# foundation-model-stack/fms-fsdp

Hardware: NVIDIA H100
Metric: tokens/sec (llama2_1.4b FSDP seq4096 bs2) (higher is better)
Workload: dtype bf16; 1 GPU; model=llama2_1.4b, global_batch=2, seq_len=4096, parallelism=fsdp1, selective_ac=0, data_stream=get_dummy_loader (arange windows mod vocab, label == input), l2=per-step working set (GBs of weights+activations) >> 50 MB L2; no explicit flush

## Files before the change

### fms_fsdp_b200/csrc/attention_sm90.cu

```cuda
#include "common.cuh"
#include "tensormap.h"
#include "wgmma.cuh"

namespace b200 {

constexpr int ATT_THREADS = 256;
constexpr float LOG2E = 1.4426950408889634f;
constexpr float LN2 = 0.6931471805599453f;

template <int HD, int TB>
B200_DEVINL void mma_rs_hd(float (&d)[HD / 2], const uint32_t (&a)[4], uint64_t bdesc) {
  if constexpr (HD == 128) wgmma_bf16_rs_n128<TB>(d, a, bdesc, 1);
  else wgmma_bf16_rs_n64<TB>(d, a, bdesc, 1);
}

template <int NREG>
B200_DEVINL void acc_to_frag(const float (&v)[NREG], int kk, uint32_t (&a)[4]) {
  a[0] = pack_bf16x2(v[8 * kk + 0], v[8 * kk + 1]);
  a[1] = pack_bf16x2(v[8 * kk + 2], v[8 * kk + 3]);
  a[2] = pack_bf16x2(v[8 * kk + 4], v[8 * kk + 5]);
  a[3] = pack_bf16x2(v[8 * kk + 6], v[8 * kk + 7]);
}

B200_DEVINL float quad_max(float v) {
// ... 357 lines not shown
    }
    wgmma_commit();
    wgmma_wait<0>();
    named_bar_sync(1, ATT_THREADS);
    if (threadIdx.x == 0 && it + 2 < n_iter) load_y(it + 2);
  }

  const int Wd = (H + 2 * KVH) * HD;
#pragma unroll
  for (int hh = 0; hh < 2; ++hh) {
    const int x = x_lo + 8 * hh;
    if (x >= S) continue;
    __nv_bfloat16* drow = dqkv + ((size_t)b * S + x) * Wd;
    const int col2 = (MODE == MODE_DKDV) ? (H + kvh) * HD : head_lo * HD;
    const float* trow = rope ? rope + (size_t)x * HD : nullptr;
#pragma unroll
    for (int jj = 0; jj < HD / 8; ++jj) {
      const int c = 8 * jj + cq;
      float f0 = acc2[4 * jj + 2 * hh] * scale, f1 = acc2[4 * jj + 2 * hh + 1] * scale;
      if (trow) {
        const float2 cs = *reinterpret_cast<const float2*>(trow + c);
        const float a0 = f0, a1 = f1;
        f0 = a0 * cs.x + a1 * cs.y;
        f1 = a1 * cs.x - a0 * cs.y;
      }
      *reinterpret_cast<uint32_t*>(drow + col2 + c) = pack_bf16x2(f0, f1);
      if constexpr (MODE == MODE_DKDV)
        *reinterpret_cast<uint32_t*>(drow + (H + KVH + kvh) * HD + c) =
            pack_bf16x2(acc1[4 * jj + 2 * hh], acc1[4 * jj + 2 * hh + 1]);
    }
  }
}

template <int HD, bool DOC>
static int launch_fwd(const void* qkv, void* o, float* lse, int B, int S, int H, int KVH, float scale, const int* seg,
                      cudaStream_t st) {
  using C = FwdCfg<HD>;
  CUtensorMap tm;
  const int W = (H + 2 * KVH) * HD;
  if (make_tmap_2d_bf16(&tm, qkv, (uint64_t)W, (uint64_t)B * S, (uint64_t)W, 64, 128)) return -3;
  auto kern = attn_fwd_kernel<HD, DOC>;
  static bool configured = false;
  if (!configured) {
    cudaError_t e = cudaFuncSetAttribute(kern, cudaFuncAttributeMaxDynamicSharedMemorySize, C::SMEM);
    if (e != cudaSuccess) return (int)e;
    configured = true;
  }
  const int n_qt = (S + 127) / 128;
  kern<<<dim3(n_qt, H, B), ATT_THREADS, C::SMEM, st>>>(tm, (__nv_bfloat16*)o, lse, S, H, KVH, scale * LOG2E, n_qt,
                                                       seg);
  return (int)cudaGetLastError();
}

template <int HD, bool DOC>
static int launch_bwd(const void* dout, const void* qkv, const void* o, const float* lse, void* dqkv, float* delta,
                      int B, int S, int H, int KVH, float scale, const float* rope, const int* seg, cudaStream_t st) {
  using C = BwdCfg<HD>;
  const int W = (H + 2 * KVH) * HD;
  CUtensorMap q64, d64;
  if (make_tmap_2d_bf16(&q64, qkv, (uint64_t)W, (uint64_t)B * S, (uint64_t)W, 64, 64)) return -3;
  if (make_tmap_2d_bf16(&d64, dout, (uint64_t)H * HD, (uint64_t)B * S, (uint64_t)H * HD, 64, 64)) return -3;
  const int ld = ((S + 127) / 128) * 128;
  float* lse2 = delta + (size_t)B * H * ld;
  {
    const long long lanes = (long long)B * S * H * (HD / 8);
    const long long blocks = (lanes + 255) / 256;
    attn_delta_kernel<HD><<<(unsigned)blocks, 256, 0, st>>>((const __nv_bfloat16*)dout, (const __nv_bfloat16*)o, delta,
                                                            lse, lse2, B, S, H, ld);
  }
  auto j1 = attn_bwd_kernel<HD, MODE_DKDV, DOC>;
  auto j2 = attn_bwd_kernel<HD, MODE_DQ, DOC>;
  static bool configured = false;
  if (!configured) {
    cudaError_t e = cudaFuncSetAttribute(j1, cudaFuncAttributeMaxDynamicSharedMemorySize, C::SMEM);
    if (e != cudaSuccess) return (int)e;
    e = cudaFuncSetAttribute(j2, cudaFuncAttributeMaxDynamicSharedMemorySize, C::SMEM);
    if (e != cudaSuccess) return (int)e;
    configured = true;
  }
  const int n_t = (S + 127) / 128;
  const int* seg1 = DOC ? seg + (size_t)B * S : nullptr;
  j1<<<dim3(n_t, KVH, B), ATT_THREADS, C::SMEM, st>>>(q64, d64, lse2, delta, (__nv_bfloat16*)dqkv, S, H, KVH, scale, n_t,
                                                      ld, rope, seg1);
  j2<<<dim3(n_t, H, B), ATT_THREADS, C::SMEM, st>>>(q64, d64, lse2, delta, (__nv_bfloat16*)dqkv, S, H, KVH, scale, n_t,
                                                    ld, rope, seg);
  return (int)cudaGetLastError();
}

}

extern "C" int b200_attn_fwd(const void* qkv, void* o, float* lse, int B, int S, int H, int KVH, int HD, float scale,
                             cudaStream_t st, const int* seg) {
  if (H % KVH) return -1;
  if (seg) {
    if (HD == 128) return b200::launch_fwd<128, true>(qkv, o, lse, B, S, H, KVH, scale, seg, st);
    if (HD == 64) return b200::launch_fwd<64, true>(qkv, o, lse, B, S, H, KVH, scale, seg, st);
    return -2;
  }
  if (HD == 128) return b200::launch_fwd<128, false>(qkv, o, lse, B, S, H, KVH, scale, nullptr, st);
  if (HD == 64) return b200::launch_fwd<64, false>(qkv, o, lse, B, S, H, KVH, scale, nullptr, st);
  return -2;
}
extern "C" int b200_attn_bwd(const void* dout, const void* qkv, const void* o, const float* lse, void* dqkv,
                             float* delta, int B, int S, int H, int KVH, int HD, float scale, const float* rope,
                             cudaStream_t st, const int* seg) {
  if (H % KVH) return -1;
  if (seg) {
    if (HD == 128) return b200::launch_bwd<128, true>(dout, qkv, o, lse, dqkv, delta, B, S, H, KVH, scale, rope, seg, st);
    if (HD == 64) return b200::launch_bwd<64, true>(dout, qkv, o, lse, dqkv, delta, B, S, H, KVH, scale, rope, seg, st);
    return -2;
  }
  if (HD == 128) return b200::launch_bwd<128, false>(dout, qkv, o, lse, dqkv, delta, B, S, H, KVH, scale, rope, nullptr, st);
  if (HD == 64) return b200::launch_bwd<64, false>(dout, qkv, o, lse, dqkv, delta, B, S, H, KVH, scale, rope, nullptr, st);
  return -2;
}
```

### fms_fsdp_b200/csrc/bindings.cpp

```cpp
#include <ATen/cuda/CUDAContext.h>
#include <c10/cuda/CUDAGuard.h>
#include <torch/extension.h>

#include <cmath>
#include <cstdint>

#define DECL extern "C"
DECL int b200_gemm_bf16(const void*, const void*, void*, const void*, int, int, int, int, int, int, int, int, int, int,
                        int, cudaStream_t);
DECL int b200_gemm2_bf16(const void*, const void*, void*, const void*, int, int, int, int, int, int, int, int, int, int,
                         int, cudaStream_t);
DECL int b200_gemm2_ag_bf16(const void*, const void*, void*, const void*, int, int, int, int, int, int, int, int, int, int,
                            const void* const*, void*, unsigned long long, unsigned long long, unsigned long long, int, int,
                            uint32_t*, uint32_t, int, cudaStream_t);
DECL int b200_bgemm_bf16(const void*, const void*, void*, int, int, int, int, int, int, int, int, long long, long long,
                         long long, long long, long long, long long, int, int, int, int, cudaStream_t);
DECL int b200_ssd_prep(const void*, const float*, const float*, float*, float*, float*, int, int, int, cudaStream_t);
DECL int b200_ssd_mask(const void*, const float*, const float*, void*, int, int, int, cudaStream_t);
DECL int b200_ssd_xs(const void*, const float*, const float*, const float*, void*, long long, int, int, cudaStream_t);
DECL int b200_ssd_state_pass(const float*, const float*, void*, int, int, int, int, int, cudaStream_t);
DECL int b200_ssd_combine(const void*, const void*, const void*, const float*, const float*, void*, long long, int, int,
                          cudaStream_t);
DECL int b200_ssd_dyoff(const void*, const void*, const void*, const float*, void*, float*, float*, long long, int,
                        cudaStream_t);
// ... 8 lines not shown
DECL int b200_selscan_fwd(const void*, const void*, const float*, const void*, const void*, const float*, const void*,
                          const float*, float*, void*, int, int, int, int, int, cudaStream_t);
DECL int b200_selscan_bwd(const void*, const void*, const void*, const float*, const void*, const void*, const float*,
                          const void*, const float*, float*, void*, void*, void*, float*, float*, float*, float*, float*, int,
                          int, int, int, int, cudaStream_t);
DECL void b200_comm_set_reduce_ctas(int);
DECL int b200_p2p_gather_range(const void* const*, void*, long long, long long, long long, cudaStream_t);
DECL int b200_rmsnorm_fwd(const void*, const void*, void*, float*, int, int, float, cudaStream_t);
DECL int b200_rmsnorm_bwd_grid(int);
DECL int b200_rmsnorm_bwd(const void*, const void*, const void*, const float*, const void*, void*, float*, float*, int, int,
                          cudaStream_t);
DECL int b200_add_rmsnorm_fwd(const void*, const float*, const void*, void*, float*, float*, int, int, float, cudaStream_t);
DECL int b200_rmsnorm_bwd_f32(const void*, const float*, const void*, const float*, float*, float*, float*, int, int, cudaStream_t);
DECL int b200_rmsnorm_gated_fwd(const void*, const void*, const void*, void*, float*, int, int, float, cudaStream_t);
DECL int b200_rmsnorm_gated_bwd(const void*, const void*, const void*, const void*, const float*, void*, void*, float*, float*, int, int, cudaStream_t);
DECL int b200_rope(void*, const float*, int, int, int, int, int, int, int, int, int, cudaStream_t);
DECL int b200_qk_norm_rope(void*, void*, float*, const void*, const void*, const float*, int, int, int, int, int, int, float,
                           cudaStream_t);
DECL int b200_qk_norm_bwd_grid(int, int, int);
DECL int b200_qk_norm_bwd(void*, const void*, const float*, const void*, const void*, float*, float*, int, int, int, int,
                          int, cudaStream_t);
DECL int b200_swiglu_fwd(const void*, void*, long long, int, int, cudaStream_t);
DECL int b200_swiglu_bwd(const void*, const void*, void*, long long, int, int, cudaStream_t);
DECL int b200_embedding_fwd(const void*, int, const void*, void*, long long, int, cudaStream_t);
DECL int b200_embedding_bwd(const void*, int, const void*, void*, int, long long, int, cudaStream_t);
DECL int b200_count_valid(const long long*, int, long long, float*, cudaStream_t);
DECL int b200_ce_grad_inplace(void*, const long long*, const float*, float*, int, int, int, long long, cudaStream_t);
DECL int b200_adamw(float*, const void*, int, float*, float*, void*, long long, float, float, float, float, float,
                    float, float, const float*, cudaStream_t);
DECL int b200_sumsq(const void*, int, long long, float*, cudaStream_t);
DECL int b200_attn_fwd(const void*, void*, float*, int, int, int, int, int, float, cudaStream_t, const int*);
DECL int b200_attn_bwd(const void*, const void*, const void*, const float*, void*, float*, int, int, int, int, int,
                       float, const float*, cudaStream_t, const int*);
DECL void b200_gemm2_set_rope(const float*, int, int, int);
DECL void b200_gemm2_set_swiglu(void*, int, int, int);
DECL void b200_gemm2_set_tile(int);
DECL int b200_gemm2_fp8(const void*, const void*, void*, const float*, const float*, int, int, int, int, int, int, cudaStream_t);
DECL int b200_quant_rowwise_e4m3(const void*, void*, float*, int, int, int, int, cudaStream_t);
DECL void b200_gemm2_set_push(void* const*, long long, long long, int, int, int);
DECL int b200_p2p_push_range(const void*, void* const*, long long, long long, long long, int, cudaStream_t);
DECL int b200_p2p_allgather(const void* const*, void*, long long, int, int, cudaStream_t);
DECL int b200_reduce_scatter(const void* const*, float*, long long, long long, int, int, int, float, float*, int,
                             cudaStream_t);
DECL int b200_allreduce_inplace(void* const*, long long, int, int, int, float, float*, cudaStream_t);
DECL int b200_signal_barrier(uint32_t* const*, int, int, uint32_t, int, int, cudaStream_t);
DECL int b200_scalar_allreduce_bytes();
DECL int b200_scalar_allreduce(uint8_t* const*, int, int, uint32_t, float*, int, cudaStream_t);
DECL int b200_gemm_grouped_bf16(const void*, const void*, void*, const int*, const int*, int, int, int, int, int, int, int,
                                int, int, int, int, cudaStream_t);
DECL int b200_moe_route(const float*, int, int, int, int, float*, int*, float*, cudaStream_t);
DECL int b200_moe_plan_ws_chunks(int);
DECL int b200_moe_plan(const int*, const float*, int, int, int, int, int*, float*, int*, int*, int*, int*, int*, float*,
                       cudaStream_t);
DECL int b200_moe_permute(const void*, const int*, const int*, const int*, const int*, int, int, int, void*, cudaStream_t);
DECL int b200_moe_permute_bwd(const void*, const int*, int, int, int, void*, cudaStream_t);
DECL int b200_moe_combine(const void*, const int*, const float*, const void*, int, int, int, void*, cudaStream_t);
DECL int b200_moe_combine_bwd(const void*, const void*, const float*, const int*, const int*, const int*, const int*, int,
                              int, int, void*, float*, cudaStream_t);
DECL int b200_moe_route_bwd(const float*, const int*, const float*, const float*, const int*, int, int, int, int, float,
                            void*, cudaStream_t);
DECL int b200_causal_conv1d_fwd(const void*, const void*, const void*, void*, int, int, int, int, int, cudaStream_t);
DECL int b200_causal_conv1d_bwd(const void*, const void*, const void*, const void*, void*, float*, float*, int, int,
                                int, int, int, cudaStream_t);

namespace {

// ... 278 lines not shown
  need(master, "master", at::kFloat);
  need(m, "m", at::kFloat);
  need(v, "v", at::kFloat);
  TORCH_CHECK(grad.scalar_type() == at::kBFloat16 || grad.scalar_type() == at::kFloat);
  TORCH_CHECK(grad.numel() == master.numel());
  void* lp = nullptr;
  if (lowp.has_value()) {
    need(*lowp, "lowp", at::kBFloat16);
    lp = lowp->data_ptr();
  }
  const float* gs = grad_scale.has_value() ? grad_scale->data_ptr<float>() : nullptr;
  const double bc1 = 1.0 - std::pow(b1, (double)step), bc2 = 1.0 - std::pow(b2, (double)step);
  check(b200_adamw(master.data_ptr<float>(), grad.data_ptr(), grad.scalar_type() == at::kBFloat16,
                   m.data_ptr<float>(), v.data_ptr<float>(), lp, master.numel(), (float)lr, (float)b1, (float)b2,
                   (float)eps, (float)wd, (float)bc1, (float)std::sqrt(bc2), gs, cur_stream()), "adamw");
}
void sumsq(const at::Tensor& x, at::Tensor& out) {
  c10::cuda::CUDAGuard guard(x.device());
  TORCH_CHECK(x.is_contiguous() && (x.scalar_type() == at::kBFloat16 || x.scalar_type() == at::kFloat));
  need(out, "out", at::kFloat);
  check(b200_sumsq(x.data_ptr(), x.scalar_type() == at::kBFloat16, x.numel(), out.data_ptr<float>(), cur_stream()),
        "sumsq");
}

const int* seg_ptr(const c10::optional<at::Tensor>& seg, const at::Tensor& qkv, int64_t B, int64_t S) {
  if (!seg.has_value() || !seg->defined()) return nullptr;
  TORCH_CHECK(seg->scalar_type() == at::kInt, "seg has dtype ", seg->scalar_type(), ", expected int32");
  TORCH_CHECK(seg->is_contiguous(), "seg must be contiguous");
  TORCH_CHECK(seg->device() == qkv.device(), "seg must be on the device of qkv");
  TORCH_CHECK(seg->numel() == 2 * B * S, "seg must be a [2, B*S] table");
  return seg->data_ptr<int>();
}

std::vector<at::Tensor> attn_fwd(const at::Tensor& qkv, int64_t B, int64_t S, int64_t H, int64_t KVH, int64_t hd,
                                 double scale, const c10::optional<at::Tensor>& seg) {
  c10::cuda::CUDAGuard guard(qkv.device());
  need(qkv, "qkv", at::kBFloat16);
  TORCH_CHECK(qkv.is_contiguous());
  const int* seg_p = seg_ptr(seg, qkv, B, S);
  auto o = at::empty({B * S, H * hd}, qkv.options());
  auto lse = at::empty({B, H, S}, qkv.options().dtype(at::kFloat));
  check(b200_attn_fwd(qkv.data_ptr(), o.data_ptr(), lse.data_ptr<float>(), B, S, H, KVH, hd, (float)scale,
                      cur_stream(), seg_p), "attn_fwd");
  return {o, lse};
}
at::Tensor attn_bwd(const at::Tensor& dout, const at::Tensor& qkv, const at::Tensor& o, const at::Tensor& lse,
                    int64_t B, int64_t S, int64_t H, int64_t KVH, int64_t hd, double scale,
                    const c10::optional<at::Tensor>& rope, const c10::optional<at::Tensor>& seg) {
  c10::cuda::CUDAGuard guard(qkv.device());
  need(qkv, "qkv", at::kBFloat16);
  need(dout, "do", at::kBFloat16);
  need(o, "o", at::kBFloat16);
  need(lse, "lse", at::kFloat);
  TORCH_CHECK(qkv.is_contiguous() && dout.is_contiguous() && o.is_contiguous() && lse.is_contiguous());
  const int* seg_p = seg_ptr(seg, qkv, B, S);
  auto dqkv = at::empty_like(qkv);
  auto delta = at::empty({2, B, H, ((S + 127) / 128) * 128}, qkv.options().dtype(at::kFloat));
  const float* rope_p = nullptr;
  if (rope.has_value() && rope->defined()) {
    need(*rope, "rope", at::kFloat);
    TORCH_CHECK(rope->is_contiguous() && rope->numel() >= S * hd, "attn_bwd: rope table must be [S, hd/2, 2] fp32");
    rope_p = rope->data_ptr<float>();
  }
  check(b200_attn_bwd(dout.data_ptr(), qkv.data_ptr(), o.data_ptr(), lse.data_ptr<float>(), dqkv.data_ptr(),
                      delta.data_ptr<float>(), B, S, H, KVH, hd, (float)scale, rope_p, cur_stream(), seg_p),
        "attn_bwd", 3);
  return dqkv;
}

void p2p_allgather(const at::Tensor& peer_ptrs, at::Tensor& full, int64_t shard_bytes, int64_t world, int64_t rank) {
  c10::cuda::CUDAGuard guard(full.device());
  check(b200_p2p_allgather((const void* const*)peer_ptrs.data_ptr(), full.data_ptr(), shard_bytes, world, rank,
                           cur_stream()), "p2p_allgather");
}
void reduce_scatter(const at::Tensor& peer_ptrs, at::Tensor& out32, int64_t elem_offset, int64_t world, int64_t rank,
                    bool src_bf16, double scale, const c10::optional<at::Tensor>& sumsq_out, int64_t max_ctas,
                    bool accumulate) {
  c10::cuda::CUDAGuard guard(out32.device());
  need(out32, "out", at::kFloat);
  b200_comm_set_reduce_ctas(max_ctas > 0 ? (int)max_ctas : g_reduce_ctas_default);
  check(b200_reduce_scatter((const void* const*)peer_ptrs.data_ptr(), out32.data_ptr<float>(), out32.numel(),
                            elem_offset, world, rank, src_bf16, (float)scale,
                            sumsq_out.has_value() ? sumsq_out->data_ptr<float>() : nullptr, accumulate ? 1 : 0,
                            cur_stream()),
        "reduce_scatter");
}
void allreduce_inplace(const at::Tensor& peer_ptrs, int64_t numel, int64_t world, int64_t rank, bool is_bf16,
                       double scale, const c10::optional<at::Tensor>& sumsq_out, const at::Tensor& anchor) {
  c10::cuda::CUDAGuard guard(anchor.device());
  check(b200_allreduce_inplace((void* const*)peer_ptrs.data_ptr(), numel, world, rank, is_bf16, (float)scale,
                               sumsq_out.has_value() ? sumsq_out->data_ptr<float>() : nullptr, cur_stream()),
        "allreduce_inplace");
}
void signal_barrier(const at::Tensor& pad_ptrs, int64_t world, int64_t rank, int64_t epoch, const at::Tensor& anchor,
                    int64_t slot_base, int64_t mode) {
  c10::cuda::CUDAGuard guard(anchor.device());
  check(b200_signal_barrier((uint32_t* const*)pad_ptrs.data_ptr(), world, rank, (uint32_t)epoch, (int)slot_base, (int)mode,
                            cur_stream()), "signal_barrier");
}
void scalar_allreduce(const at::Tensor& buf_ptrs, int64_t world, int64_t rank, int64_t epoch, at::Tensor& inout) {
// ... 490 lines not shown
PYBIND11_MODULE(TORCH_EXTENSION_NAME, m) {
  m.doc() = "fms_fsdp_b200 sm_90a kernels";
  m.def("gemm", &gemm);
  m.def("gemm_grouped", &gemm_grouped);
  m.def("moe_route", &moe_route);
  m.def("moe_plan", &moe_plan);
  m.def("moe_permute", &moe_permute);
  m.def("moe_permute_bwd", &moe_permute_bwd);
  m.def("moe_combine", &moe_combine);
  m.def("moe_combine_bwd", &moe_combine_bwd);
  m.def("moe_route_bwd", &moe_route_bwd);
  m.def("rmsnorm_fwd", &rmsnorm_fwd);
  m.def("rmsnorm_bwd", &rmsnorm_bwd, py::arg("dy"), py::arg("x"), py::arg("w"), py::arg("rstd"), py::arg("dres") = py::none());
  m.def("add_rmsnorm_fwd", &add_rmsnorm_fwd);
  m.def("rmsnorm_bwd_f32", &rmsnorm_bwd_f32);
  m.def("rmsnorm_gated_fwd", &rmsnorm_gated_fwd);
  m.def("rmsnorm_gated_bwd", &rmsnorm_gated_bwd);
  m.def("rope", &rope);
  m.def("qk_norm_rope", &qk_norm_rope);
  m.def("qk_norm_bwd", &qk_norm_bwd);
  m.def("swiglu_fwd", &swiglu_fwd);
  m.def("swiglu_bwd", &swiglu_bwd);
  m.def("embedding_fwd", &embedding_fwd);
  m.def("embedding_bwd", &embedding_bwd);
  m.def("count_valid", &count_valid);
  m.def("ce_grad_inplace", &ce_grad_inplace);
  m.def("adamw", &adamw);
  m.def("sumsq", &sumsq);
  m.def("attn_fwd", &attn_fwd, py::arg("qkv"), py::arg("B"), py::arg("S"), py::arg("H"), py::arg("KVH"), py::arg("hd"),
        py::arg("scale"), py::arg("seg") = py::none());
  m.def("attn_bwd", &attn_bwd, py::arg("dout"), py::arg("qkv"), py::arg("o"), py::arg("lse"), py::arg("B"), py::arg("S"),
        py::arg("H"), py::arg("KVH"), py::arg("hd"), py::arg("scale"), py::arg("rope") = py::none(),
        py::arg("seg") = py::none());
  m.def("p2p_allgather", &p2p_allgather);
  m.def("reduce_scatter", &reduce_scatter, py::arg("peer_ptrs"), py::arg("out32"), py::arg("elem_offset"), py::arg("world"),
        py::arg("rank"), py::arg("src_bf16"), py::arg("scale"), py::arg("sumsq_out"), py::arg("max_ctas") = 0,
        py::arg("accumulate") = false);
  m.def("allreduce_inplace", &allreduce_inplace);
  m.def("signal_barrier", &signal_barrier, py::arg("pad_ptrs"), py::arg("world"), py::arg("rank"), py::arg("epoch"),
        py::arg("anchor"), py::arg("slot_base") = 0, py::arg("mode") = 0);
  m.def("scalar_allreduce", &scalar_allreduce);
  m.def("scalar_allreduce_bytes", []() { return (int64_t)b200_scalar_allreduce_bytes(); });
  m.def("causal_conv1d_fwd", &causal_conv1d_fwd);
  m.def("causal_conv1d_bwd", &causal_conv1d_bwd);
  m.def("set_reduce_ctas", [](int64_t n) { g_reduce_ctas_default = n < 1 ? 1 : (int)n; b200_comm_set_reduce_ctas((int)n); });
  m.def("set_gemm_rope", [](const at::Tensor& table, int64_t S, int64_t hd, int64_t cols) {
    need(table, "rope table", at::kFloat);
    TORCH_CHECK(table.is_contiguous() && table.numel() >= S * hd, "rope table must be [S, hd/2, 2] fp32");
    b200_gemm2_set_rope(table.data_ptr<float>(), (int)S, (int)hd, (int)cols);
  });
  m.def("push_range", [](const at::Tensor& src, const at::Tensor& bases, int64_t n, int64_t off, int64_t rank) {
    c10::cuda::CUDAGuard guard(src.device());
    need(src, "src", at::kBFloat16);
    TORCH_CHECK(src.is_contiguous() && bases.scalar_type() == at::kLong && bases.is_cuda());
    check(b200_p2p_push_range(src.data_ptr(), (void* const*)bases.data_ptr(), n, off, src.numel(), (int)rank, cur_stream()),
          "p2p_push_range");
  });
  m.def("set_gemm_swiglu", [](const at::Tensor& aux, int64_t F, bool gate_first) {
    need(aux, "aux", at::kBFloat16);
    TORCH_CHECK(aux.dim() == 2 && aux.stride(1) == 1 && (aux.size(1) == F || aux.size(1) == 2 * F));
    b200_gemm2_set_swiglu(aux.data_ptr(), (int)aux.stride(0), (int)F, gate_first ? 1 : 0);
  });
  m.def("set_gemm_push", [](const at::Tensor& bases, int64_t n, int64_t off, int64_t rank, bool bulk, int64_t rot_world) {
    TORCH_CHECK(bases.is_cuda() && bases.scalar_type() == at::kLong && bases.is_contiguous(), "push table: int64 CUDA tensor");
    b200_gemm2_set_push((void* const*)bases.data_ptr(), n, off, (int)rank, bulk ? 1 : 0, (int)rot_world);
  }, py::arg("bases"), py::arg("n"), py::arg("off"), py::arg("rank"), py::arg("bulk") = true, py::arg("rot_world") = 1);
// ... 16 lines not shown
```

Baseline: 49640 tokens/s.

## Add warp-specialized TMA producer/consumer pipelined attention forward and backward kernels

Adds new forward and backward attention kernels that dedicate one warpgroup to TMA loads (with setmaxnreg register reallocation) and two consumer warpgroups that run wgmma. K/V tiles are multi-buffered with full/empty mbarriers, and the forward overlaps the next QK^T with the current PV product. The default entry points now dispatch to the pipelined path, and the old kernels stay reachable through new lockstep bindings. This is meant to hide load latency and keep the tensor cores busy, at the cost of higher shared-memory and register pressure and one CTA per SM.

Result: faster. 52770 tokens/s, median of 6 (+6.3%).

```diff
diff --git a/fms_fsdp_b200/csrc/attention_sm90.cu b/fms_fsdp_b200/csrc/attention_sm90.cu
--- a/fms_fsdp_b200/csrc/attention_sm90.cu
+++ b/fms_fsdp_b200/csrc/attention_sm90.cu
@@ -413,30 +413,464 @@
   }
 }
 
+constexpr int PIPE_THREADS = 384;
+constexpr int PRODUCER_REGS = 24, CONSUMER_REGS = 240;
+
+template <int N>
+B200_DEVINL void attn_regs_dec() { asm volatile("setmaxnreg.dec.sync.aligned.u32 %0;" ::"n"(N)); }
+template <int N>
+B200_DEVINL void attn_regs_inc() { asm volatile("setmaxnreg.inc.sync.aligned.u32 %0;" ::"n"(N)); }
+
+B200_DEVINL void bulk_load_1d(void* dst, const void* src, uint32_t bytes, uint64_t* bar) {
+  asm volatile("cp.async.bulk.shared::cluster.global.mbarrier::complete_tx::bytes [%0], [%1], %2, [%3];"
+               ::"r"(smem_u32(dst)), "l"(reinterpret_cast<uint64_t>(src)), "r"(bytes), "r"(smem_u32(bar))
+               : "memory");
+}
+
+template <int HD>
+struct FwdPipeCfg {
+  static constexpr int NCH = HD / 64;
+  static constexpr int TILE_BYTES = 128 * HD * 2;
+  static constexpr int STAGES = 2;
+  static constexpr int SMEM = TILE_BYTES * (1 + 2 * STAGES) + 1024 + 256;
+};
+
 template <int HD, bool DOC>
+__global__ void __launch_bounds__(PIPE_THREADS, 1)
+attn_fwd_pipe_kernel(const __grid_constant__ CUtensorMap tm, __nv_bfloat16* __restrict__ o, float* __restrict__ lse,
+                     int S, int H, int KVH, float scale_log2, int n_qt, const int* __restrict__ seg0) {
+  using C = FwdPipeCfg<HD>;
+  constexpr int ST = C::STAGES;
+  extern __shared__ uint8_t smem_raw[];
+  uint8_t* smem = reinterpret_cast<uint8_t*>((reinterpret_cast<uintptr_t>(smem_raw) + 1023) & ~uintptr_t(1023));
+  uint8_t* sQ = smem;
+  uint8_t* sK = sQ + C::TILE_BYTES;
+  uint8_t* sV = sK + ST * C::TILE_BYTES;
+  uint64_t* bars = reinterpret_cast<uint64_t*>(sV + ST * C::TILE_BYTES);
+  uint64_t* q_full = bars;
+  uint64_t* k_full = bars + 1;
+  uint64_t* v_full = k_full + ST;
+  uint64_t* k_empty = v_full + ST;
+  uint64_t* v_empty = k_empty + ST;
+
+  const int wg = threadIdx.x >> 7, w4 = (threadIdx.x >> 5) & 3, lane = threadIdx.x & 31;
+  const int h = blockIdx.x, b = blockIdx.y;
+  const int qt = n_qt - 1 - blockIdx.z;
+  const int kvh = h / (H / KVH);
+  const int row0 = b * S + qt * 128;
+  const int n_kv = min(qt + 1, (S + 127) / 128);
+  const int* srow = DOC ? seg0 + static_cast<size_t>(b) * S : nullptr;
+  const int j_lo = DOC ? srow[qt * 128] / 128 : 0;
+
+  if (threadIdx.x == 0) {
+    mbar_init(q_full, 1);
+    for (int s = 0; s < ST; ++s) {
+      mbar_init(&k_full[s], 1);
+      mbar_init(&v_full[s], 1);
+      mbar_init(&k_empty[s], 8);
+      mbar_init(&v_empty[s], 8);
+    }
+    fence_barrier_init();
+  }
+  __syncthreads();
+
+  if (wg == 0) {
+    attn_regs_dec<PRODUCER_REGS>();
+    if (threadIdx.x == 0) {
+      tma_prefetch_desc(&tm);
+      mbar_arrive_expect_tx(q_full, C::TILE_BYTES);
+      for (int c = 0; c < C::NCH; ++c) tma_load_2d(sQ + c * 16384, &tm, q_full, h * HD + 64 * c, row0);
+      for (int j = j_lo; j < n_kv; ++j) {
+        const int st = (j - j_lo) % ST;
+        const uint32_t ph = ((j - j_lo) / ST) & 1;
+        const int krow = b * S + j * 128;
+        mbar_wait(&k_empty[st], ph ^ 1);
+        mbar_arrive_expect_tx(&k_full[st], C::TILE_BYTES);
+        for (int c = 0; c < C::NCH; ++c)
+          tma_load_2d(sK + st * C::TILE_BYTES + c * 16384, &tm, &k_full[st], (H + kvh) * HD + 64 * c, krow);
+        mbar_wait(&v_empty[st], ph ^ 1);
+        mbar_arrive_expect_tx(&v_full[st], C::TILE_BYTES);
+        for (int c = 0; c < C::NCH; ++c)
+          tma_load_2d(sV + st * C::TILE_BYTES + c * 16384, &tm, &v_full[st], (H + KVH + kvh) * HD + 64 * c, krow);
+      }
+    }
+    asm volatile("exit;");
+  }
+  attn_regs_inc<CONSUMER_REGS>();
+  const int cw = wg - 1;
+
+  const int r_lo = qt * 128 + cw * 64 + w4 * 16 + (lane >> 2);
+  const int cq = 2 * (lane & 3);
+  int doc_lo[2] = {0, 0}, tile_doc_hi = 0;
+  if constexpr (DOC) {
+    doc_lo[0] = srow[min(r_lo, S - 1)];
+    doc_lo[1] = srow[min(r_lo + 8, S - 1)];
+    tile_doc_hi = srow[min(qt * 128 + 127, S - 1)];
+  }
+  const uint64_t qd = make_smem_desc(smem_u32(sQ) + cw * 8192, 0, 1024);
+  float oacc[HD / 2];
+#pragma unroll
+  for (int i = 0; i < HD / 2; ++i) oacc[i] = 0.f;
+  float m_run[2] = {-INFINITY, -INFINITY}, l_run[2] = {0.f, 0.f};
+
+  auto issue_s = [&](int j, float (&s)[64]) {
+    const int n = j - j_lo;
+    mbar_wait(&k_full[n % ST], (n / ST) & 1);
+    const uint64_t kd = make_smem_desc(smem_u32(sK + (n % ST) * C::TILE_BYTES), 0, 1024);
+    wgmma_fence();
+#pragma unroll
+    for (int kk = 0; kk < HD / 16; ++kk) {
+      const uint32_t off = ((kk >> 2) * 16384 + (kk & 3) * 32) >> 4;
+      wgmma_bf16_ss_n128<0, 0>(s, qd + off, kd + off, kk != 0);
+    }
+    wgmma_commit();
+  };
+  auto issue_pv = [&](int j, const uint32_t (&pa)[8][4]) {
+    const int n = j - j_lo;
+    mbar_wait(&v_full[n % ST], (n / ST) & 1);
+    const uint64_t vd = make_smem_desc(smem_u32(sV + (n % ST) * C::TILE_BYTES), 16384, 1024);
+    wgmma_fence();
+#pragma unroll
+    for (int kk = 0; kk < 8; ++kk) mma_rs_hd<HD, 1>(oacc, pa[kk], vd + ((kk * 2048) >> 4));
+    wgmma_commit();
+  };
+  auto release = [&](uint64_t* empty, int j) {
+    if (lane == 0) mbar_arrive(&empty[(j - j_lo) % ST]);
+  };
+  auto softmax = [&](int j, float (&s)[64], float (&corr)[2]) {
+    const int kv0 = j * 128;
+    if (j == qt || kv0 + 128 > S || (DOC && kv0 < tile_doc_hi)) {
+#pragma unroll
+      for (int i = 0; i < 64; ++i) {
+        const int kv = kv0 + 8 * (i >> 2) + cq + (i & 1);
+        const int q = r_lo + 8 * ((i >> 1) & 1);
+        if (kv > q || kv >= S || (DOC && kv < doc_lo[(i >> 1) & 1])) s[i] = -INFINITY;
+      }
+    }
+#pragma unroll
+    for (int hh = 0; hh < 2; ++hh) {
+      float mx = -INFINITY;
+#pragma unroll
+      for (int jj = 0; jj < 16; ++jj) mx = fmaxf(mx, fmaxf(s[4 * jj + 2 * hh], s[4 * jj + 2 * hh + 1]));
+      const float m_new = fmaxf(m_run[hh], quad_max(mx) * scale_log2);
+      const float m_sub = (DOC && m_new == -INFINITY) ? 0.f : m_new;
+      corr[hh] = exp2f(m_run[hh] - m_sub);
+      m_run[hh] = m_new;
+      float ls = 0.f;
+#pragma unroll
+      for (int jj = 0; jj < 16; ++jj) {
+#pragma unroll
+        for (int e = 0; e < 2; ++e) {
+          const int i = 4 * jj + 2 * hh + e;
+          s[i] = exp2f(fmaf(s[i], scale_log2, -m_sub));
+          ls += s[i];
+        }
+      }
+      l_run[hh] = l_run[hh] * corr[hh] + ls;
+    }
+  };
+
+  mbar_wait(q_full, 0);
+  float s[64], corr[2];
+  uint32_t pa[8][4];
+  issue_s(j_lo, s);
+  wgmma_wait<0>();
+  release(k_empty, j_lo);
+  softmax(j_lo, s, corr);
+#pragma unroll
+  for (int i = 0; i < HD / 2; ++i) oacc[i] *= corr[(i >> 1) & 1];
+#pragma unroll
+  for (int kk = 0; kk < 8; ++kk) acc_to_frag(s, kk, pa[kk]);
+  for (int j = j_lo + 1; j < n_kv; ++j) {
+    issue_s(j, s);
+    issue_pv(j - 1, pa);
+    wgmma_wait<1>();
+    release(k_empty, j);
+    softmax(j, s, corr);
+    wgmma_wait<0>();
+    release(v_empty, j - 1);
+#pragma unroll
+    for (int i = 0; i < HD / 2; ++i) oacc[i] *= corr[(i >> 1) & 1];
+#pragma unroll
+    for (int kk = 0; kk < 8; ++kk) acc_to_frag(s, kk, pa[kk]);
+  }
+  issue_pv(n_kv - 1, pa);
+  wgmma_wait<0>();
+
+#pragma unroll
+  for (int hh = 0; hh < 2; ++hh) {
+    const int q = r_lo + 8 * hh;
+    const float l = quad_sum(l_run[hh]);
+    if (q < S) {
+      const float inv_l = 1.f / l;
+      __nv_bfloat16* orow = o + (static_cast<size_t>(b) * S + q) * (H * HD) + h * HD;
+#pragma unroll
+      for (int jj = 0; jj < HD / 8; ++jj)
+        *reinterpret_cast<uint32_t*>(orow + 8 * jj + cq) =
+            pack_bf16x2(oacc[4 * jj + 2 * hh] * inv_l, oacc[4 * jj + 2 * hh + 1] * inv_l);
+      if ((lane & 3) == 0) lse[(static_cast<size_t>(b) * H + h) * S + q] = (m_run[hh] + log2f(l)) * LN2;
+    }
+  }
+}
+
+template <int HD>
+struct BwdPipeCfg {
+  static constexpr int NCH = HD / 64;
+  static constexpr int X_BYTES = 128 * HD * 2;
+  static constexpr int Y_BYTES = 64 * HD * 2;
+  static constexpr int STAGES = 3;
+  static constexpr int STAT_BYTES = 2 * 64 * 4;
+  static constexpr int SMEM = 2 * X_BYTES + STAGES * (2 * Y_BYTES + STAT_BYTES) + 1024 + 256;
+};
+
+template <int HD, int MODE, bool DOC>
+__global__ void __launch_bounds__(PIPE_THREADS, 1)
+attn_bwd_pipe_kernel(const __grid_constant__ CUtensorMap tm_qkv, const __grid_constant__ CUtensorMap tm_do,
+                     const float* __restrict__ lse2g, const float* __restrict__ delta, __nv_bfloat16* __restrict__ dqkv,
+                     int S, int H, int KVH, float scale, int n_t128, int ld, const float* __restrict__ rope,
+                     const int* __restrict__ seg_plane) {
+  using C = BwdPipeCfg<HD>;
+  constexpr int ST = C::STAGES;
+  extern __shared__ uint8_t smem_raw[];
+  uint8_t* smem = reinterpret_cast<uint8_t*>((reinterpret_cast<uintptr_t>(smem_raw) + 1023) & ~uintptr_t(1023));
+  uint8_t* sX1 = smem;
+  uint8_t* sX2 = sX1 + C::X_BYTES;
+  uint8_t* sY = sX2 + C::X_BYTES;
+  float* sStat = reinterpret_cast<float*>(sY + ST * 2 * C::Y_BYTES);
+  uint64_t* bars = reinterpret_cast<uint64_t*>(sStat + ST * 128);
+  uint64_t* x_full = bars;
+  uint64_t* y_full = bars + 1;
+  uint64_t* y_empty = y_full + ST;
+
+  const int wg = threadIdx.x >> 7, w4 = (threadIdx.x >> 5) & 3, lane = threadIdx.x & 31;
+  const int G = H / KVH;
+  const int b = blockIdx.y;
+  const float scale_log2 = scale * LOG2E;
+  const int n_t64 = (S + 63) / 64;
+  int t128, head_lo, head_n, kvh;
+  if constexpr (MODE == MODE_DKDV) {
+    t128 = blockIdx.z; kvh = blockIdx.x; head_lo = kvh * G; head_n = G;
+  } else {
+    t128 = n_t128 - 1 - blockIdx.z; head_lo = blockIdx.x; head_n = 1; kvh = blockIdx.x / G;
+  }
+  const int* srow = DOC ? seg_plane + static_cast<size_t>(b) * S : nullptr;
+  const int tile_doc_first = DOC ? srow[t128 * 128] : 0;
+  const int tile_doc_last = DOC ? srow[min(t128 * 128 + 127, S - 1)] : 0;
+  const int s_lo = (MODE == MODE_DKDV) ? 2 * t128 : (DOC ? tile_doc_first / 64 : 0);
+  const int s_hi = (MODE == MODE_DKDV) ? (DOC ? tile_doc_last / 64 + 1 : n_t64) : min(2 * t128 + 2, n_t64);
+  const int per_head = s_hi - s_lo;
+  const int n_iter = per_head * head_n;
+  const int xrow0 = b * S + t128 * 128;
+
+  if (threadIdx.x == 0) {
+    mbar_init(x_full, 1);
+    for (int s = 0; s < ST; ++s) {
+      mbar_init(&y_full[s], 1);
+      mbar_init(&y_empty[s], 8);
+    }
+    fence_barrier_init();
+  }
+  __syncthreads();
+
+  if (wg == 0) {
+    attn_regs_dec<PRODUCER_REGS>();
+    if (threadIdx.x == 0) {
+      tma_prefetch_desc(&tm_qkv); tma_prefetch_desc(&tm_do);
+      mbar_arrive_expect_tx(x_full, 2 * C::X_BYTES);
+      for (int c = 0; c < C::NCH; ++c) {
+        for (int half = 0; half < 2; ++half) {
+          uint8_t* d1 = sX1 + c * 16384 + half * 8192;
+          uint8_t* d2 = sX2 + c * 16384 + half * 8192;
+          const int r = xrow0 + 64 * half;
+          if constexpr (MODE == MODE_DKDV) {
+            tma_load_2d(d1, &tm_qkv, x_full, (H + kvh) * HD + 64 * c, r);
+            tma_load_2d(d2, &tm_qkv, x_full, (H + KVH + kvh) * HD + 64 * c, r);
+          } else {
+            tma_load_2d(d1, &tm_qkv, x_full, head_lo * HD + 64 * c, r);
+            tma_load_2d(d2, &tm_do, x_full, head_lo * HD + 64 * c, r);
+          }
+        }
+      }
+      for (int it = 0; it < n_iter; ++it) {
+        const int st = it % ST;
+        const int hh = head_lo + it / per_head;
+        const int y0 = (s_lo + it % per_head) * 64;
+        uint8_t* y1 = sY + st * 2 * C::Y_BYTES;
+        uint8_t* y2 = y1 + C::Y_BYTES;
+        mbar_wait(&y_empty[st], ((it / ST) & 1) ^ 1);
+        mbar_arrive_expect_tx(&y_full[st], 2 * C::Y_BYTES + (MODE == MODE_DKDV ? C::STAT_BYTES : 0));
+        for (int c = 0; c < C::NCH; ++c) {
+          if constexpr (MODE == MODE_DKDV) {
+            tma_load_2d(y1 + c * 8192, &tm_qkv, &y_full[st], hh * HD + 64 * c, b * S + y0);
+            tma_load_2d(y2 + c * 8192, &tm_do, &y_full[st], hh * HD + 64 * c, b * S + y0);
+          } else {
+            tma_load_2d(y1 + c * 8192, &tm_qkv, &y_full[st], (H + kvh) * HD + 64 * c, b * S + y0);
+            tma_load_2d(y2 + c * 8192, &tm_qkv, &y_full[st], (H + KVH + kvh) * HD + 64 * c, b * S + y0);
+          }
+        }
+        if constexpr (MODE == MODE_DKDV) {
+          const size_t base = ((size_t)b * H + hh) * ld + y0;
+          bulk_load_1d(sStat + st * 128, lse2g + base, 256, &y_full[st]);
+          bulk_load_1d(sStat + st * 128 + 64, delta + base, 256, &y_full[st]);
+        }
+      }
+    }
+    asm volatile("exit;");
+  }
+  attn_regs_inc<CONSUMER_REGS>();
+  const int cw = wg - 1;
+
+  const int x_lo = t128 * 128 + cw * 64 + w4 * 16 + (lane >> 2);
+  const int cq = 2 * (lane & 3);
+  const uint64_t x1d = make_smem_desc(smem_u32(sX1) + cw * 8192, 0, 1024);
+  const uint64_t x2d = make_smem_desc(smem_u32(sX2) + cw * 8192, 0, 1024);
+  float acc1[MODE == MODE_DKDV ? HD / 2 : 1];
+  float acc2[HD / 2];
+#pragma unroll
+  for (int i = 0; i < HD / 2; ++i) acc2[i] = 0.f;
+#pragma unroll
+  for (int i = 0; i < (MODE == MODE_DKDV ? HD / 2 : 1); ++i) acc1[i] = 0.f;
+  float row_nl[2] = {0.f, 0.f}, row_nd[2] = {0.f, 0.f};
+  int row_doc[2] = {0, 0};
+  if constexpr (DOC) {
+    row_doc[0] = srow[min(x_lo, S - 1)];
+    row_doc[1] = srow[min(x_lo + 8, S - 1)];
+  }
+  if constexpr (MODE == MODE_DQ) {
+#pragma unroll
+    for (int hh = 0; hh < 2; ++hh) {
+      const size_t sidx = ((size_t)b * H + head_lo) * ld + min(x_lo + 8 * hh, S - 1);
+      row_nl[hh] = lse2g[sidx];
+      row_nd[hh] = delta[sidx];
+    }
+  }
+
+  constexpr bool CARRY = !(MODE == MODE_DKDV && HD == 128);
+  mbar_wait(x_full, 0);
+  uint32_t pa[4][4], da[4][4];
+  for (int it = 0; it < n_iter; ++it) {
+    const int st = it % ST;
+    const int y0 = (s_lo + it % per_head) * 64;
+    const uint32_t y1a = smem_u32(sY + st * 2 * C::Y_BYTES), y2a = y1a + C::Y_BYTES;
+    mbar_wait(&y_full[st], (it / ST) & 1);
+    const uint64_t y1d = make_smem_desc(y1a, 0, 1024), y2d = make_smem_desc(y2a, 0, 1024);
+    float s[32], dp[32];
+    wgmma_fence();
+#pragma unroll
+    for (int kk = 0; kk < HD / 16; ++kk) {
+      const uint32_t ox = ((kk >> 2) * 16384 + (kk & 3) * 32) >> 4, oy = ((kk >> 2) * 8192 + (kk & 3) * 32) >> 4;
+      wgmma_bf16_ss_n64<0, 0>(s, x1d + ox, y1d + oy, kk != 0);
+    }
+    wgmma_commit();
+#pragma unroll
+    for (int kk = 0; kk < HD / 16; ++kk) {
+      const uint32_t ox = ((kk >> 2) * 16384 + (kk & 3) * 32) >> 4, oy = ((kk >> 2) * 8192 + (kk & 3) * 32) >> 4;
+      wgmma_bf16_ss_n64<0, 0>(dp, x2d + ox, y2d + oy, kk != 0);
+    }
+    wgmma_commit();
+    wgmma_wait<1>();
+    if (CARRY && it > 0 && lane == 0) mbar_arrive(&y_empty[(it - 1) % ST]);
+    const bool diag = (MODE == MODE_DKDV) ? (y0 < t128 * 128 + 128) : (y0 + 64 > t128 * 128);
+    const bool doc_edge = DOC && ((MODE == MODE_DKDV) ? (y0 + 63 > tile_doc_first) : (y0 < tile_doc_last));
+    const bool need_mask = diag || (y0 + 64 > S) || (t128 * 128 + 128 > S) || doc_edge;
+    const float* stl = sStat + st * 128;
+    uint32_t mbits = 0;
+#pragma unroll
+    for (int i = 0; i < 32; ++i) {
+      const int x = x_lo + 8 * ((i >> 1) & 1);
+      const int y = y0 + 8 * (i >> 2) + cq + (i & 1);
+      const float nl = (MODE == MODE_DKDV) ? stl[8 * (i >> 2) + cq + (i & 1)] : row_nl[(i >> 1) & 1];
+      bool masked = false;
+      if (need_mask) masked = (MODE == MODE_DKDV) ? (x > y || y >= S || x >= S) : (y > x || y >= S || x >= S);
+      if constexpr (DOC) {
+        const int bound = row_doc[(i >> 1) & 1];
+        if (need_mask) masked = masked || ((MODE == MODE_DKDV) ? (y > bound) : (y < bound));
+      }
+      mbits |= (masked ? 1u : 0u) << i;
+      s[i] = masked ? 0.f : exp2f(fmaf(s[i], scale_log2, nl));
+    }
+    const uint64_t y1t = make_smem_desc(y1a, 8192, 1024), y2t = make_smem_desc(y2a, 8192, 1024);
+    if constexpr (MODE == MODE_DKDV) {
+#pragma unroll
+      for (int kk = 0; kk < 4; ++kk) acc_to_frag(s, kk, pa[kk]);
+      wgmma_fence();
+#pragma unroll
+      for (int kk = 0; kk < 4; ++kk) mma_rs_hd<HD, 1>(acc1, pa[kk], y2t + ((kk * 2048) >> 4));
+      wgmma_commit();
+      wgmma_wait<1>();
+    } else {
+      wgmma_wait<0>();
+    }
+#pragma unroll
+    for (int i = 0; i < 32; ++i) {
+      const float nd = (MODE == MODE_DKDV) ? stl[64 + 8 * (i >> 2) + cq + (i & 1)] : row_nd[(i >> 1) & 1];
+      dp[i] = ((mbits >> i) & 1u) ? 0.f : s[i] * (dp[i] + nd);
+    }
+#pragma unroll
+    for (int kk = 0; kk < 4; ++kk) acc_to_frag(dp, kk, da[kk]);
+    wgmma_fence();
+#pragma unroll
+    for (int kk = 0; kk < 4; ++kk) mma_rs_hd<HD, 1>(acc2, da[kk], y1t + ((kk * 2048) >> 4));
+    wgmma_commit();
+    if constexpr (!CARRY) {
+      wgmma_wait<0>();
+      if (lane == 0) mbar_arrive(&y_empty[st]);
+    }
+  }
+  wgmma_wait<0>();
+
+  const int Wd = (H + 2 * KVH) * HD;
+#pragma unroll
+  for (int hh = 0; hh < 2; ++hh) {
+    const int x = x_lo + 8 * hh;
+    if (x >= S) continue;
+    __nv_bfloat16* drow = dqkv + ((size_t)b * S + x) * Wd;
+    const int col2 = (MODE == MODE_DKDV) ? (H + kvh) * HD : head_lo * HD;
+    const float* trow = rope ? rope + (size_t)x * HD : nullptr;
+#pragma unroll
+    for (int jj = 0; jj < HD / 8; ++jj) {
+      const int c = 8 * jj + cq;
+      float f0 = acc2[4 * jj + 2 * hh] * scale, f1 = acc2[4 * jj + 2 * hh + 1] * scale;
+      if (trow) {
+        const float2 cs = *reinterpret_cast<const float2*>(trow + c);
+        const float a0 = f0, a1 = f1;
+        f0 = a0 * cs.x + a1 * cs.y;
+        f1 = a1 * cs.x - a0 * cs.y;
+      }
+      *reinterpret_cast<uint32_t*>(drow + col2 + c) = pack_bf16x2(f0, f1);
+      if constexpr (MODE == MODE_DKDV)
+        *reinterpret_cast<uint32_t*>(drow + (H + KVH + kvh) * HD + c) =
+            pack_bf16x2(acc1[4 * jj + 2 * hh], acc1[4 * jj + 2 * hh + 1]);
+    }
+  }
+}
+
+template <int HD, bool DOC, bool PIPE>
 static int launch_fwd(const void* qkv, void* o, float* lse, int B, int S, int H, int KVH, float scale, const int* seg,
                       cudaStream_t st) {
-  using C = FwdCfg<HD>;
+  constexpr int SMEM = PIPE ? FwdPipeCfg<HD>::SMEM : FwdCfg<HD>::SMEM;
   CUtensorMap tm;
   const int W = (H + 2 * KVH) * HD;
   if (make_tmap_2d_bf16(&tm, qkv, (uint64_t)W, (uint64_t)B * S, (uint64_t)W, 64, 128)) return -3;
-  auto kern = attn_fwd_kernel<HD, DOC>;
+  auto kern = PIPE ? attn_fwd_pipe_kernel<HD, DOC> : attn_fwd_kernel<HD, DOC>;
   static bool configured = false;
   if (!configured) {
-    cudaError_t e = cudaFuncSetAttribute(kern, cudaFuncAttributeMaxDynamicSharedMemorySize, C::SMEM);
+    cudaError_t e = cudaFuncSetAttribute(kern, cudaFuncAttributeMaxDynamicSharedMemorySize, SMEM);
     if (e != cudaSuccess) return (int)e;
     configured = true;
   }
   const int n_qt = (S + 127) / 128;
-  kern<<<dim3(n_qt, H, B), ATT_THREADS, C::SMEM, st>>>(tm, (__nv_bfloat16*)o, lse, S, H, KVH, scale * LOG2E, n_qt,
-                                                       seg);
+  if constexpr (PIPE)
+    kern<<<dim3(H, B, n_qt), PIPE_THREADS, SMEM, st>>>(tm, (__nv_bfloat16*)o, lse, S, H, KVH, scale * LOG2E, n_qt, seg);
+  else
+    kern<<<dim3(n_qt, H, B), ATT_THREADS, SMEM, st>>>(tm, (__nv_bfloat16*)o, lse, S, H, KVH, scale * LOG2E, n_qt, seg);
   return (int)cudaGetLastError();
 }
 
-template <int HD, bool DOC>
+template <int HD, bool DOC, bool PIPE>
 static int launch_bwd(const void* dout, const void* qkv, const void* o, const float* lse, void* dqkv, float* delta,
                       int B, int S, int H, int KVH, float scale, const float* rope, const int* seg, cudaStream_t st) {
-  using C = BwdCfg<HD>;
+  constexpr int SMEM = PIPE ? BwdPipeCfg<HD>::SMEM : BwdCfg<HD>::SMEM;
   const int W = (H + 2 * KVH) * HD;
   CUtensorMap q64, d64;
   if (make_tmap_2d_bf16(&q64, qkv, (uint64_t)W, (uint64_t)B * S, (uint64_t)W, 64, 64)) return -3;
@@ -449,49 +883,70 @@
     attn_delta_kernel<HD><<<(unsigned)blocks, 256, 0, st>>>((const __nv_bfloat16*)dout, (const __nv_bfloat16*)o, delta,
                                                             lse, lse2, B, S, H, ld);
   }
-  auto j1 = attn_bwd_kernel<HD, MODE_DKDV, DOC>;
-  auto j2 = attn_bwd_kernel<HD, MODE_DQ, DOC>;
+  auto j1 = PIPE ? attn_bwd_pipe_kernel<HD, MODE_DKDV, DOC> : attn_bwd_kernel<HD, MODE_DKDV, DOC>;
+  auto j2 = PIPE ? attn_bwd_pipe_kernel<HD, MODE_DQ, DOC> : attn_bwd_kernel<HD, MODE_DQ, DOC>;
   static bool configured = false;
   if (!configured) {
-    cudaError_t e = cudaFuncSetAttribute(j1, cudaFuncAttributeMaxDynamicSharedMemorySize, C::SMEM);
+    cudaError_t e = cudaFuncSetAttribute(j1, cudaFuncAttributeMaxDynamicSharedMemorySize, SMEM);
     if (e != cudaSuccess) return (int)e;
-    e = cudaFuncSetAttribute(j2, cudaFuncAttributeMaxDynamicSharedMemorySize, C::SMEM);
+    e = cudaFuncSetAttribute(j2, cudaFuncAttributeMaxDynamicSharedMemorySize, SMEM);
     if (e != cudaSuccess) return (int)e;
     configured = true;
   }
   const int n_t = (S + 127) / 128;
   const int* seg1 = DOC ? seg + (size_t)B * S : nullptr;
-  j1<<<dim3(n_t, KVH, B), ATT_THREADS, C::SMEM, st>>>(q64, d64, lse2, delta, (__nv_bfloat16*)dqkv, S, H, KVH, scale, n_t,
-                                                      ld, rope, seg1);
-  j2<<<dim3(n_t, H, B), ATT_THREADS, C::SMEM, st>>>(q64, d64, lse2, delta, (__nv_bfloat16*)dqkv, S, H, KVH, scale, n_t,
-                                                    ld, rope, seg);
+  const dim3 g1 = PIPE ? dim3(KVH, B, n_t) : dim3(n_t, KVH, B), g2 = PIPE ? dim3(H, B, n_t) : dim3(n_t, H, B);
+  const int threads = PIPE ? PIPE_THREADS : ATT_THREADS;
+  j1<<<g1, threads, SMEM, st>>>(q64, d64, lse2, delta, (__nv_bfloat16*)dqkv, S, H, KVH, scale, n_t, ld, rope, seg1);
+  j2<<<g2, threads, SMEM, st>>>(q64, d64, lse2, delta, (__nv_bfloat16*)dqkv, S, H, KVH, scale, n_t, ld, rope, seg);
   return (int)cudaGetLastError();
+}
+
+template <bool PIPE>
+static int attn_fwd(const void* qkv, void* o, float* lse, int B, int S, int H, int KVH, int HD, float scale,
+                    cudaStream_t st, const int* seg) {
+  if (H % KVH) return -1;
+  if (seg) {
+    if (HD == 128) return launch_fwd<128, true, PIPE>(qkv, o, lse, B, S, H, KVH, scale, seg, st);
+    if (HD == 64) return launch_fwd<64, true, PIPE>(qkv, o, lse, B, S, H, KVH, scale, seg, st);
+    return -2;
+  }
+  if (HD == 128) return launch_fwd<128, false, PIPE>(qkv, o, lse, B, S, H, KVH, scale, nullptr, st);
+  if (HD == 64) return launch_fwd<64, false, PIPE>(qkv, o, lse, B, S, H, KVH, scale, nullptr, st);
+  return -2;
+}
+
+template <bool PIPE>
+static int attn_bwd(const void* dout, const void* qkv, const void* o, const float* lse, void* dqkv, float* delta, int B,
+                    int S, int H, int KVH, int HD, float scale, const float* rope, cudaStream_t st, const int* seg) {
+  if (H % KVH) return -1;
+  if (seg) {
+    if (HD == 128) return launch_bwd<128, true, PIPE>(dout, qkv, o, lse, dqkv, delta, B, S, H, KVH, scale, rope, seg, st);
+    if (HD == 64) return launch_bwd<64, true, PIPE>(dout, qkv, o, lse, dqkv, delta, B, S, H, KVH, scale, rope, seg, st);
+    return -2;
+  }
+  if (HD == 128) return launch_bwd<128, false, PIPE>(dout, qkv, o, lse, dqkv, delta, B, S, H, KVH, scale, rope, nullptr, st);
+  if (HD == 64) return launch_bwd<64, false, PIPE>(dout, qkv, o, lse, dqkv, delta, B, S, H, KVH, scale, rope, nullptr, st);
+  return -2;
 }
 
 }
 
 extern "C" int b200_attn_fwd(const void* qkv, void* o, float* lse, int B, int S, int H, int KVH, int HD, float scale,
                              cudaStream_t st, const int* seg) {
-  if (H % KVH) return -1;
-  if (seg) {
-    if (HD == 128) return b200::launch_fwd<128, true>(qkv, o, lse, B, S, H, KVH, scale, seg, st);
-    if (HD == 64) return b200::launch_fwd<64, true>(qkv, o, lse, B, S, H, KVH, scale, seg, st);
-    return -2;
-  }
-  if (HD == 128) return b200::launch_fwd<128, false>(qkv, o, lse, B, S, H, KVH, scale, nullptr, st);
-  if (HD == 64) return b200::launch_fwd<64, false>(qkv, o, lse, B, S, H, KVH, scale, nullptr, st);
-  return -2;
+  return b200::attn_fwd<true>(qkv, o, lse, B, S, H, KVH, HD, scale, st, seg);
 }
 extern "C" int b200_attn_bwd(const void* dout, const void* qkv, const void* o, const float* lse, void* dqkv,
                              float* delta, int B, int S, int H, int KVH, int HD, float scale, const float* rope,
                              cudaStream_t st, const int* seg) {
-  if (H % KVH) return -1;
-  if (seg) {
-    if (HD == 128) return b200::launch_bwd<128, true>(dout, qkv, o, lse, dqkv, delta, B, S, H, KVH, scale, rope, seg, st);
-    if (HD == 64) return b200::launch_bwd<64, true>(dout, qkv, o, lse, dqkv, delta, B, S, H, KVH, scale, rope, seg, st);
-    return -2;
-  }
-  if (HD == 128) return b200::launch_bwd<128, false>(dout, qkv, o, lse, dqkv, delta, B, S, H, KVH, scale, rope, nullptr, st);
-  if (HD == 64) return b200::launch_bwd<64, false>(dout, qkv, o, lse, dqkv, delta, B, S, H, KVH, scale, rope, nullptr, st);
-  return -2;
-}
+  return b200::attn_bwd<true>(dout, qkv, o, lse, dqkv, delta, B, S, H, KVH, HD, scale, rope, st, seg);
+}
+extern "C" int b200_attn_fwd_lockstep(const void* qkv, void* o, float* lse, int B, int S, int H, int KVH, int HD,
+                                      float scale, cudaStream_t st, const int* seg) {
+  return b200::attn_fwd<false>(qkv, o, lse, B, S, H, KVH, HD, scale, st, seg);
+}
+extern "C" int b200_attn_bwd_lockstep(const void* dout, const void* qkv, const void* o, const float* lse, void* dqkv,
+                                      float* delta, int B, int S, int H, int KVH, int HD, float scale, const float* rope,
+                                      cudaStream_t st, const int* seg) {
+  return b200::attn_bwd<false>(dout, qkv, o, lse, dqkv, delta, B, S, H, KVH, HD, scale, rope, st, seg);
+}
diff --git a/fms_fsdp_b200/csrc/bindings.cpp b/fms_fsdp_b200/csrc/bindings.cpp
--- a/fms_fsdp_b200/csrc/bindings.cpp
+++ b/fms_fsdp_b200/csrc/bindings.cpp
@@ -64,6 +64,9 @@
 DECL int b200_attn_fwd(const void*, void*, float*, int, int, int, int, int, float, cudaStream_t, const int*);
 DECL int b200_attn_bwd(const void*, const void*, const void*, const float*, void*, float*, int, int, int, int, int,
                        float, const float*, cudaStream_t, const int*);
+DECL int b200_attn_fwd_lockstep(const void*, void*, float*, int, int, int, int, int, float, cudaStream_t, const int*);
+DECL int b200_attn_bwd_lockstep(const void*, const void*, const void*, const float*, void*, float*, int, int, int, int,
+                                int, float, const float*, cudaStream_t, const int*);
 DECL void b200_gemm2_set_rope(const float*, int, int, int);
 DECL void b200_gemm2_set_swiglu(void*, int, int, int);
 DECL void b200_gemm2_set_tile(int);
@@ -408,21 +411,24 @@
   return seg->data_ptr<int>();
 }
 
-std::vector<at::Tensor> attn_fwd(const at::Tensor& qkv, int64_t B, int64_t S, int64_t H, int64_t KVH, int64_t hd,
-                                 double scale, const c10::optional<at::Tensor>& seg) {
+using AttnFwdFn = decltype(&b200_attn_fwd);
+using AttnBwdFn = decltype(&b200_attn_bwd);
+static std::vector<at::Tensor> attn_fwd_with(AttnFwdFn fn, const at::Tensor& qkv, int64_t B, int64_t S, int64_t H,
+                                             int64_t KVH, int64_t hd, double scale, const c10::optional<at::Tensor>& seg) {
   c10::cuda::CUDAGuard guard(qkv.device());
   need(qkv, "qkv", at::kBFloat16);
   TORCH_CHECK(qkv.is_contiguous());
   const int* seg_p = seg_ptr(seg, qkv, B, S);
   auto o = at::empty({B * S, H * hd}, qkv.options());
   auto lse = at::empty({B, H, S}, qkv.options().dtype(at::kFloat));
-  check(b200_attn_fwd(qkv.data_ptr(), o.data_ptr(), lse.data_ptr<float>(), B, S, H, KVH, hd, (float)scale,
-                      cur_stream(), seg_p), "attn_fwd");
+  check(fn(qkv.data_ptr(), o.data_ptr(), lse.data_ptr<float>(), B, S, H, KVH, hd, (float)scale, cur_stream(), seg_p),
+        "attn_fwd");
   return {o, lse};
 }
-at::Tensor attn_bwd(const at::Tensor& dout, const at::Tensor& qkv, const at::Tensor& o, const at::Tensor& lse,
-                    int64_t B, int64_t S, int64_t H, int64_t KVH, int64_t hd, double scale,
-                    const c10::optional<at::Tensor>& rope, const c10::optional<at::Tensor>& seg) {
+static at::Tensor attn_bwd_with(AttnBwdFn fn, const at::Tensor& dout, const at::Tensor& qkv, const at::Tensor& o,
+                                const at::Tensor& lse, int64_t B, int64_t S, int64_t H, int64_t KVH, int64_t hd,
+                                double scale, const c10::optional<at::Tensor>& rope,
+                                const c10::optional<at::Tensor>& seg) {
   c10::cuda::CUDAGuard guard(qkv.device());
   need(qkv, "qkv", at::kBFloat16);
   need(dout, "do", at::kBFloat16);
@@ -438,10 +444,28 @@
     TORCH_CHECK(rope->is_contiguous() && rope->numel() >= S * hd, "attn_bwd: rope table must be [S, hd/2, 2] fp32");
     rope_p = rope->data_ptr<float>();
   }
-  check(b200_attn_bwd(dout.data_ptr(), qkv.data_ptr(), o.data_ptr(), lse.data_ptr<float>(), dqkv.data_ptr(),
-                      delta.data_ptr<float>(), B, S, H, KVH, hd, (float)scale, rope_p, cur_stream(), seg_p),
+  check(fn(dout.data_ptr(), qkv.data_ptr(), o.data_ptr(), lse.data_ptr<float>(), dqkv.data_ptr(),
+           delta.data_ptr<float>(), B, S, H, KVH, hd, (float)scale, rope_p, cur_stream(), seg_p),
         "attn_bwd", 3);
   return dqkv;
+}
+std::vector<at::Tensor> attn_fwd(const at::Tensor& qkv, int64_t B, int64_t S, int64_t H, int64_t KVH, int64_t hd,
+                                 double scale, const c10::optional<at::Tensor>& seg) {
+  return attn_fwd_with(b200_attn_fwd, qkv, B, S, H, KVH, hd, scale, seg);
+}
+at::Tensor attn_bwd(const at::Tensor& dout, const at::Tensor& qkv, const at::Tensor& o, const at::Tensor& lse,
+                    int64_t B, int64_t S, int64_t H, int64_t KVH, int64_t hd, double scale,
+                    const c10::optional<at::Tensor>& rope, const c10::optional<at::Tensor>& seg) {
+  return attn_bwd_with(b200_attn_bwd, dout, qkv, o, lse, B, S, H, KVH, hd, scale, rope, seg);
+}
+std::vector<at::Tensor> attn_fwd_lockstep(const at::Tensor& qkv, int64_t B, int64_t S, int64_t H, int64_t KVH,
+                                          int64_t hd, double scale, const c10::optional<at::Tensor>& seg) {
+  return attn_fwd_with(b200_attn_fwd_lockstep, qkv, B, S, H, KVH, hd, scale, seg);
+}
+at::Tensor attn_bwd_lockstep(const at::Tensor& dout, const at::Tensor& qkv, const at::Tensor& o, const at::Tensor& lse,
+                             int64_t B, int64_t S, int64_t H, int64_t KVH, int64_t hd, double scale,
+                             const c10::optional<at::Tensor>& rope, const c10::optional<at::Tensor>& seg) {
+  return attn_bwd_with(b200_attn_bwd_lockstep, dout, qkv, o, lse, B, S, H, KVH, hd, scale, rope, seg);
 }
 
 void p2p_allgather(const at::Tensor& peer_ptrs, at::Tensor& full, int64_t shard_bytes, int64_t world, int64_t rank) {
@@ -998,6 +1022,11 @@
   m.def("attn_bwd", &attn_bwd, py::arg("dout"), py::arg("qkv"), py::arg("o"), py::arg("lse"), py::arg("B"), py::arg("S"),
         py::arg("H"), py::arg("KVH"), py::arg("hd"), py::arg("scale"), py::arg("rope") = py::none(),
         py::arg("seg") = py::none());
+  m.def("attn_fwd_lockstep", &attn_fwd_lockstep, py::arg("qkv"), py::arg("B"), py::arg("S"), py::arg("H"),
+        py::arg("KVH"), py::arg("hd"), py::arg("scale"), py::arg("seg") = py::none());
+  m.def("attn_bwd_lockstep", &attn_bwd_lockstep, py::arg("dout"), py::arg("qkv"), py::arg("o"), py::arg("lse"),
+        py::arg("B"), py::arg("S"), py::arg("H"), py::arg("KVH"), py::arg("hd"), py::arg("scale"),
+        py::arg("rope") = py::none(), py::arg("seg") = py::none());
   m.def("p2p_allgather", &p2p_allgather);
   m.def("reduce_scatter", &reduce_scatter, py::arg("peer_ptrs"), py::arg("out32"), py::arg("elem_offset"), py::arg("world"),
         py::arg("rank"), py::arg("src_bf16"), py::arg("scale"), py::arg("sumsq_out"), py::arg("max_ctas") = 0,
```
